# m96-chan/PyGPUkit

Measured on AMD Instinct MI355X. Metric: decode tokens/sec/GPU + prefill TFLOPS (% MFMA peak), Qwen3-0.6B bf16, higher is better.
Workload: dtype bf16

## Files before the change

pygpukit_amd/csrc/attn_core.hip.h:

```cpp
#pragma once

#include <type_traits>

#include "attn_plan.h"
#include "pgk_device.hip.h"

#ifdef PGK_PHASE_STAMPS
static __device__ unsigned long long* g_phase_tl;
#define PGK_PHASE(i)                                                                                              \
    do {                                                                                                          \
        unsigned long long* p_ = g_phase_tl;                                                                      \
        const unsigned wg_ = blockIdx.x + gridDim.x * (blockIdx.y + gridDim.y * blockIdx.z);                      \
        if (p_ && threadIdx.x == 0 && wg_ < 256u) p_[2 * (256 + 4 * wg_) + (i)] = __builtin_amdgcn_s_memrealtime(); \
    } while (0)
#else
#define PGK_PHASE(i)
#endif

namespace pgk {

template <class T> struct KVLoad;
template <> struct KVLoad<bf16> {
    __device__ static __forceinline__ void load8(const bf16* p, float (&f)[8]) {
        Vec<bf16> v; v.load(p); v.to_float(f);
// ... 186 lines not shown
        KVBatch<U> kb;
        kv_issue<D, U, NWV>(kb, kbase, vbase, p0, c1 - 1, lane);
        kv_consume<D, G, U, NWV>(kb, p0, c1, qb, lane, st);
    }
}

template <int D, int G>
__device__ __forceinline__ void decode_block_merge(const DecodeState<G>& st, float* lds, float* part,
                                                   size_t head_stride, int lane, int wid) {
    constexpr int LPR = D / 8, PPW = 64 / LPR, NS = 4 * PPW, RS = D + 2;
    const int grp = lane / LPR, sub = lane % LPR;
    const int slot = wid * PPW + grp;
#pragma unroll
    for (int g = 0; g < G; ++g) {
        float* rec = lds + ((size_t)slot * G + g) * RS;
        if (sub == 0) { rec[0] = st.m[g]; rec[1] = st.l[g]; }
#pragma unroll
        for (int j = 0; j < 8; ++j) rec[2 + sub * 8 + j] = st.o[g][j];
    }
    __syncthreads();
    for (int e = threadIdx.x; e < G * D; e += blockDim.x) {
        const int g = e / D, d = e % D;
        float mx = -INFINITY;
        for (int s = 0; s < NS; ++s) mx = fmaxf(mx, lds[((size_t)s * G + g) * RS]);
        float l = 0.f, o = 0.f;
        for (int s = 0; s < NS; ++s) {
            const float* rec = lds + ((size_t)s * G + g) * RS;
            const float w = (rec[0] == -INFINITY) ? 0.f : __expf(rec[0] - mx);
            l = fmaf(rec[1], w, l);
            o = fmaf(rec[2 + d], w, o);
        }
        float* outrec = part + (size_t)g * head_stride;
        outrec[2 + d] = o;
        if (d == 0) { outrec[0] = mx; outrec[1] = l; }
    }
}

template <int D, int G, int NWV = 4>
__device__ __forceinline__ void decode_block_merge_lds(const DecodeState<G>& st, float* lds, float* attn_out, int lane,
                                                       int wid) {
    constexpr int LPR = D / 8, PPW = 64 / LPR, NS = NWV * PPW, RS = D + 2;
    const int grp = lane / LPR, sub = lane % LPR;
    const int slot = wid * PPW + grp;
#pragma unroll
    for (int g = 0; g < G; ++g) {
        float* rec = lds + ((size_t)slot * G + g) * RS;
        if (sub == 0) { rec[0] = st.m[g]; rec[1] = st.l[g]; }
#pragma unroll
// ... 131 lines not shown
```

pygpukit_amd/csrc/engine.hip:

```cpp

#include "engine_attn.hip.h"
#include "engine_gemv.hip.h"
#include "pkgemm.hip.h"

namespace pgk {

__global__ void embed_kernel(const bf16* embed, const int32_t* tokens, float* h, int H, const int32_t* positions,
                             const float* rope_cos, const float* rope_sin, float* cur_cos, float* cur_sin, int half,
                             int max_seq) {
    const int b = blockIdx.x;
    const bf16* row = embed + (size_t)tokens[b] * H;
    for (int i = threadIdx.x; i < H; i += blockDim.x) h[(size_t)b * H + i] = to_f(row[i]);
    const int pos = min(positions[b], max_seq - 1);
    for (int i = threadIdx.x; i < half; i += blockDim.x) {
        cur_cos[(size_t)b * half + i] = rope_cos[(size_t)pos * half + i];
        cur_sin[(size_t)b * half + i] = rope_sin[(size_t)pos * half + i];
    }
}

__global__ __launch_bounds__(256) void finalize_kernel(unsigned long long* tl, const float* amax_val, const int* amax_idx, int nblk,
                                                       int32_t* tokens, int32_t* positions, int32_t* token_log,
                                                       int32_t* step_counter, int log_width, int log_cap,
                                                       const bf16* embed, float* h, int H, int bump,
                                                       unsigned long long* clk_log, const float* rope_cos,
// ... 373 lines not shown
        while (rows < rpp) rows *= 2;
        const bool tiles = rows % rpp == 0 && c.hidden_size % rows == 0 && gd / 8 <= 64;
        e->short_path = env_on("PGK_FUSED_ATTN");
        e->fused_attn = tiles && c.weight_format == 0 && (G == 1 || G == 2 || G == 4);
        e->oproj_rows = rows;
        e->attn_mfma = c.head_dim == 128 && env_on("PGK_ATTN_MFMA");
        const int nwt = c.weight_format != 0 ? 16 : 8, lpw = gd / nwt, rpp2 = lpw > 0 ? 256 / lpw : 256;
        int rows2 = c.hidden_size / 32;
        while (rows2 > 4 * rpp2 && rows2 % 2 == 0) rows2 /= 2;
        while (rows2 < rpp2) rows2 *= 2;
        e->merged_oproj = env_on("PGK_MERGED_OPROJ") && (G == 1 || G == 2 || G == 4) && lpw >= 8 && lpw <= 64 && 256 % lpw == 0 &&
                          rows2 % rpp2 == 0 && c.hidden_size % rows2 == 0 && (c.weight_format == 0 || (gd % 128 == 0 || 128 % gd == 0)) &&
                          c.weight_format != 3;
        e->moproj_rows = rows2;
    }
    const int B = c.max_batch, H = c.hidden_size, D = c.head_dim;
    pgk_status r = PGK_OK;
    auto A = [&](void** p, size_t bytes, size_t* acct) { if (r == PGK_OK) r = dev_alloc(e, p, bytes, acct); };
    const size_t kvb = (size_t)c.num_layers * e->kv_layer_elems() * sizeof(bf16);
    A((void**)&e->kcache, kvb, &e->kv_bytes);
    A((void**)&e->vcache, kvb, &e->kv_bytes);
    A((void**)&e->rope_cos, (size_t)c.max_seq_len * (D / 2) * 4, &e->ws_bytes);
    A((void**)&e->rope_sin, (size_t)c.max_seq_len * (D / 2) * 4, &e->ws_bytes);
    A((void**)&e->cur_cos, (size_t)B * (D / 2) * 4, &e->ws_bytes);
    A((void**)&e->cur_sin, (size_t)B * (D / 2) * 4, &e->ws_bytes);
    A((void**)&e->tokens, (size_t)B * 4, &e->ws_bytes);
    A((void**)&e->positions, (size_t)B * 4, &e->ws_bytes);
    A((void**)&e->token_log, (size_t)e->log_cap * B * 4, &e->ws_bytes);
    A((void**)&e->step_counter, 16, &e->ws_bytes);
    A((void**)&e->h, (size_t)B * H * 4, &e->ws_bytes);
    A((void**)&e->h2, (size_t)B * H * 4, &e->ws_bytes);
    A((void**)&e->qkv, (size_t)B * e->qkv_dim() * 4, &e->ws_bytes);
    A((void**)&e->part, (size_t)B * c.num_heads * e->nsplit * (D + 2) * 4, &e->ws_bytes);
    A((void**)&e->opart, (size_t)B * c.num_kv_heads * H * 4, &e->ws_bytes);
    A((void**)&e->act16, (size_t)B * c.intermediate_size * 2, &e->ws_bytes);
    A((void**)&e->attnv16, (size_t)B * c.num_heads * c.head_dim * 2, &e->ws_bytes);
    A((void**)&e->x16, (size_t)B * H * 2, &e->ws_bytes);
    A((void**)&e->ss_part, (size_t)64 * 1024 * 4, &e->ws_bytes);
    A((void**)&e->attnv, (size_t)B * c.num_heads * D * 4, &e->ws_bytes);
    A((void**)&e->act, (size_t)B * c.intermediate_size * 4, &e->ws_bytes);
    A((void**)&e->logits, (size_t)B * c.vocab_size * 4, &e->ws_bytes);
    e->lm_cap = e->lm_blocks > ceil_div(c.vocab_size, 16) ? e->lm_blocks : ceil_div(c.vocab_size, 16);
    {
        const char* ev = getenv("PGK_BATCHED_MFMA");
        e->batched_min = (ev && atoi(ev) == 2) ? 3 : 5;
        auto k_ok = [](int K) { return K % 128 == 0 && K <= 4096; };
        e->batched_mfma = !(ev && atoi(ev) == 0) && k_ok(c.hidden_size) && k_ok(c.intermediate_size) && k_ok(c.num_heads * c.head_dim) &&
                          c.weight_format != 3;
// ... 519 lines not shown
```

pygpukit_amd/csrc/engine_attn.hip.h:

```cpp
#pragma once

#include "attn_core.hip.h"
#include "engine_state.hip.h"

namespace pgk {

struct AttnArgs {
    const float* qkv;
    int qkv_ld;
    const bf16 *q_gamma, *k_gamma;
    float eps;
    const float *rope_cos, *rope_sin;
    bf16 *kcache, *vcache;
    const int32_t* positions;
    int hq, hkv, max_seq;
    int span;
    float scale;
    float* part;
    int nsplit;
    float* attn_direct;
    const bf16* w_o;
    const bf16* w_o_scale;
    int H, rows_per_block;
    float* opart;
    bf16* attn_direct16;
    int g_total, g_off;
};

template <int D, int G>
struct NewToken {
    float qf[G][8], kn[8], vn[8];
    uint4 qb[G], kbits, vbits;
};

template <int G>
struct NewTokenRaw {
    float4 lo[G + 2], hi[G + 2];
    uint4 gq, gk;
    float4 cs[2], sn[2];
};

template <int D, int G>
__device__ __forceinline__ void new_token_load(const AttnArgs& a, int b, int kvh, int lane, NewTokenRaw<G>& r) {
    constexpr int LPR = D / 8, HALF = D / 2;
    const int sub = lane % LPR;
    const float* row = a.qkv + (size_t)b * a.qkv_ld;
#pragma unroll
    for (int g = 0; g < G + 2; ++g) {
        const unsigned eoff = (g < G) ? (unsigned)(kvh * a.g_total + a.g_off + g) * D : (g == G ? (unsigned)(a.hq + kvh) * D : (unsigned)(a.hq + a.hkv + kvh) * D);
        r.lo[g] = *reinterpret_cast<const float4*>(row + eoff + sub * 8);
        r.hi[g] = *reinterpret_cast<const float4*>(row + eoff + sub * 8 + 4);
    }
    r.gq = r.gk = make_uint4(0, 0, 0, 0);
    if (a.q_gamma != nullptr) {
        r.gq = *reinterpret_cast<const uint4*>(a.q_gamma + sub * 8);
        r.gk = *reinterpret_cast<const uint4*>(a.k_gamma + sub * 8);
    }
    const int dd = (sub * 8) % HALF;
    const float* cs = a.rope_cos + (size_t)b * HALF + dd;
    const float* sn = a.rope_sin + (size_t)b * HALF + dd;
    r.cs[0] = *reinterpret_cast<const float4*>(cs); r.cs[1] = *reinterpret_cast<const float4*>(cs + 4);
    r.sn[0] = *reinterpret_cast<const float4*>(sn); r.sn[1] = *reinterpret_cast<const float4*>(sn + 4);
}

template <int D, int G>
__device__ __forceinline__ void new_token_finish(const AttnArgs& a, int lane, const NewTokenRaw<G>& r, NewToken<D, G>& t) {
    constexpr int LPR = D / 8;
    const int sub = lane % LPR;
    float raw[G + 2][8], gq[8], gk[8];
#pragma unroll
    for (int g = 0; g < G + 2; ++g) {
        raw[g][0] = r.lo[g].x; raw[g][1] = r.lo[g].y; raw[g][2] = r.lo[g].z; raw[g][3] = r.lo[g].w;
        raw[g][4] = r.hi[g].x; raw[g][5] = r.hi[g].y; raw[g][6] = r.hi[g].z; raw[g][7] = r.hi[g].w;
    }
    const bool has_norm = a.q_gamma != nullptr;
    if (has_norm) {
        WTraits<bf16>::decode(r.gq, gq);
        WTraits<bf16>::decode(r.gk, gk);
    } else {
#pragma unroll
        for (int j = 0; j < 8; ++j) gq[j] = gk[j] = 1.f;
    }
    const float csv[8] = {r.cs[0].x, r.cs[0].y, r.cs[0].z, r.cs[0].w, r.cs[1].x, r.cs[1].y, r.cs[1].z, r.cs[1].w};
    const float snv[8] = {r.sn[0].x, r.sn[0].y, r.sn[0].z, r.sn[0].w, r.sn[1].x, r.sn[1].y, r.sn[1].z, r.sn[1].w};
    auto norm_rope = [&](const float (&xin)[8], const float (&gamma)[8], float (&o)[8]) {
        float x[8];
#pragma unroll
        for (int j = 0; j < 8; ++j) x[j] = xin[j];
        if (has_norm) {
            float ss = 0.f;
#pragma unroll
            for (int j = 0; j < 8; ++j) ss = fmaf(x[j], x[j], ss);
            ss = group_sum<LPR>(ss);
            const float inv = 1.0f / sqrtf(ss / D + a.eps);
#pragma unroll
            for (int j = 0; j < 8; ++j) x[j] = x[j] * inv * gamma[j];
        }
        const bool lo = sub < LPR / 2;
#pragma unroll
        for (int j = 0; j < 8; ++j) {
            const float other = xor_half<LPR>(x[j]);
            o[j] = lo ? (x[j] * csv[j] - other * snv[j]) : (x[j] * csv[j] + other * snv[j]);
        }
    };
#pragma unroll
    for (int g = 0; g < G; ++g) {
        norm_rope(raw[g], gq, t.qf[g]);
#pragma unroll
        for (int j = 0; j < 8; ++j) t.qf[g][j] *= a.scale;
        Vec<bf16> qv;
        qv.from_float(t.qf[g]);
        qv.to_float(t.qf[g]);
        t.qb[g] = qv.raw;
    }
    norm_rope(raw[G], gk, t.kn);
#pragma unroll
    for (int j = 0; j < 8; ++j) t.vn[j] = raw[G + 1][j];
    Vec<bf16> kb, vb;
    kb.from_float(t.kn);
    vb.from_float(t.vn);
    kb.to_float(t.kn);
    vb.to_float(t.vn);
    t.kbits = kb.raw;
    t.vbits = vb.raw;
}

template <int D, int G>
__device__ __forceinline__ void prepare_new_token(const AttnArgs& a, int b, int kvh, int pos, int lane, NewToken<D, G>& t) {
    NewTokenRaw<G> r;
    new_token_load<D, G>(a, b, kvh, lane, r);
    new_token_finish<D, G>(a, lane, r, t);
}

template <int D, int G>
__device__ __forceinline__ void fold_new_token(const NewToken<D, G>& t, DecodeState<G>& st) {
    constexpr int LPR = D / 8;
    float s[G];
#pragma unroll
    for (int g = 0; g < G; ++g) {
        float dsum = 0.f;
#pragma unroll
        for (int j = 0; j < 8; ++j) dsum = fmaf(t.qf[g][j], t.kn[j], dsum);
        dsum = group_sum<LPR>(dsum);
        s[g] = dsum;
    }
    st.update(s, t.vn);
}

template <int D, int G, bool DIRECT>
__global__ __launch_bounds__(256) void attn_decode_kernel(unsigned long long* tl, AttnArgs a) {
    const TLStamp tls(tl);
    constexpr int LPR = D / 8, PPW = 64 / LPR, RS = D + 2;
    __shared__ __attribute__((aligned(16))) float lds[4 * PPW * G * RS];
    __shared__ float attn_out[DIRECT ? G * D : 1];
    const int lane = threadIdx.x & 63, wid = threadIdx.x >> 6, sub = lane % LPR;
    const int kvh = blockIdx.y, b = blockIdx.z;
    const size_t head_off = (((size_t)b * a.hkv + kvh) * a.max_seq) * D;
    if constexpr (DIRECT) {
        constexpr int U0 = 8, UB = 4;
        NewTokenRaw<G> raw;
        new_token_load<D, G>(a, b, kvh, lane, raw);
        __builtin_amdgcn_sched_barrier(0);
        KVBatch<U0> kb0;
        kv_issue<D, U0, 4>(kb0, a.kcache + head_off, a.vcache + head_off, wid * PPW, a.max_seq - 1, lane);
        __builtin_amdgcn_sched_barrier(0);
        const int pos = load_uniform_i32(a.positions + b);
        const int c1 = min(pos, a.max_seq);
        KVBatch<UB> kb1;
        kv_issue<D, UB, 4>(kb1, a.kcache + head_off, a.vcache + head_off, U0 * 4 * PPW + wid * PPW, max(c1 - 1, 0), lane);
        __builtin_amdgcn_sched_barrier(0);
        NewToken<D, G> t;
        new_token_finish<D, G>(a, lane, raw, t);
        if (pos < a.max_seq && wid == 0 && lane < LPR && a.g_off == 0) {
            *reinterpret_cast<uint4*>(a.kcache + head_off + (size_t)pos * D + sub * 8) = t.kbits;
            *reinterpret_cast<uint4*>(a.vcache + head_off + (size_t)pos * D + sub * 8) = t.vbits;
        }
        DecodeState<G> st;
        st.init();
        kv_consume<D, G, U0, 4>(kb0, wid * PPW, c1, t.qb, lane, st);
        kv_consume<D, G, UB, 4>(kb1, U0 * 4 * PPW + wid * PPW, c1, t.qb, lane, st);
        if (c1 > (U0 + UB) * 4 * PPW) decode_walk_trips<D, G>(a.kcache + head_off, a.vcache + head_off, (U0 + UB) * 4 * PPW, c1, t.qb, lane, wid, st);
        if (pos < a.max_seq && wid == 0 && lane < LPR) fold_new_token<D, G>(t, st);
        decode_block_merge_lds<D, G>(st, lds, attn_out, lane, wid);
        if (a.attn_direct16) {
            for (int e = threadIdx.x; e < G * D; e += 256) a.attn_direct16[((size_t)b * a.hq + (size_t)kvh * a.g_total + a.g_off) * D + e] = from_f<bf16>(attn_out[e]);
        } else {
            for (int e = threadIdx.x; e < G * D; e += 256) a.attn_direct[((size_t)b * a.hq + (size_t)kvh * a.g_total + a.g_off) * D + e] = attn_out[e];
        }
        tls.end();
        return;
    }
    constexpr int U1 = 8;
    const int chunk = decode_chunk_len(a.span, a.nsplit, 4 * PPW);
    const int c0 = (int)blockIdx.x * chunk;
    NewTokenRaw<G> raw;
    new_token_load<D, G>(a, b, kvh, lane, raw);
    __builtin_amdgcn_sched_barrier(0);
    KVBatch<U1> kb0;
    kv_issue<D, U1, 4>(kb0, a.kcache + head_off, a.vcache + head_off, c0 + wid * PPW, a.max_seq - 1, lane);
    __builtin_amdgcn_sched_barrier(0);
    const int pos = load_uniform_i32(a.positions + b);
    const int ctx = min(pos + 1, a.max_seq);
    tls.phase(0);
    NewToken<D, G> t;
    new_token_finish<D, G>(a, lane, raw, t);
    tls.phase(1);
    const bool last_slice = (int)blockIdx.x == a.nsplit - 1;
    const int c1 = last_slice ? ctx : min(c0 + chunk, ctx);
    const bool owns_new = (pos < a.max_seq) && (pos >= c0) && (last_slice || pos < c0 + chunk);
    if (owns_new && wid == 0 && lane < LPR && a.g_off == 0) {
        *reinterpret_cast<uint4*>(a.kcache + head_off + (size_t)pos * D + sub * 8) = t.kbits;
        *reinterpret_cast<uint4*>(a.vcache + head_off + (size_t)pos * D + sub * 8) = t.vbits;
    }
    DecodeState<G> st;
    st.init();
    const int cend = owns_new ? min(c1, pos) : c1;
    kv_consume<D, G, U1, 4>(kb0, c0 + wid * PPW, cend, t.qb, lane, st);
    if (cend > c0 + U1 * 4 * PPW)
        decode_walk_trips<D, G>(a.kcache + head_off, a.vcache + head_off, c0 + U1 * 4 * PPW, cend, t.qb, lane, wid, st);
    if (owns_new && wid == 0 && lane < LPR) fold_new_token<D, G>(t, st);
    tls.phase(2);
    if constexpr (DIRECT) {
        decode_block_merge_lds<D, G>(st, lds, attn_out, lane, wid);
        for (int e = threadIdx.x; e < G * D; e += 256) a.attn_direct[((size_t)b * a.hq + (size_t)kvh * a.g_total + a.g_off) * D + e] = attn_out[e];
    } else {
        decode_block_merge<D, G>(st, lds, a.part + (((size_t)b * a.hq + (size_t)kvh * a.g_total + a.g_off) * a.nsplit + blockIdx.x) * RS,
                                 (size_t)a.nsplit * RS, lane, wid);
    }
    tls.end();
}

template <int D>
__global__ void attn_merge_kernel(unsigned long long* tl, const float* part, float* attn, int hq, int nsplit) {
    const TLStamp tls(tl);
    __shared__ float w_s[64];
    __shared__ float inv_l;
    const int h = blockIdx.x, b = blockIdx.y, d = threadIdx.x;
    const float* recs = part + ((size_t)b * hq + h) * nsplit * (D + 2);
    if (threadIdx.x < 64) {
        const int s = threadIdx.x;
        const int sc = min(s, nsplit - 1);
        float m = recs[(size_t)sc * (D + 2)], l = recs[(size_t)sc * (D + 2) + 1];
        if (s >= nsplit) { m = -INFINITY; l = 0.f; }
        const float mx = wave_max(m);
        const float w = (m == -INFINITY) ? 0.f : __expf(m - mx);
        const float tot = wave_sum(w * l);
        w_s[s] = w;
        if (s == 0) inv_l = tot > 0.f ? 1.0f / tot : 0.f;
    }
    __syncthreads();
    float o = 0.f;
// ... 415 lines not shown
                uint4 w = (p < PRE) ? pre[p < PRE ? p : 0] : load_nt16(wbase + (size_t)row * ldw);
                float wf[8];
                WTraits<bf16>::decode(w, wf);
                float acc = 0.f;
#pragma unroll
                for (int j = 0; j < 8; ++j) acc = fmaf(wf[j], xf[j], acc);
                acc = group_sum<LPW>(acc);
                if (lr == 0) outp[row] = acc;
            }
        }
    } else {
        const size_t ob = ((size_t)b * a.hq + (size_t)kvh * G) * D;
        if (a.attn_direct16) {
            for (int e = threadIdx.x; e < GD; e += 256) a.attn_direct16[ob + e] = from_f<bf16>(attn[e]);
        } else {
            for (int e = threadIdx.x; e < GD; e += 256) a.attn_direct[ob + e] = attn[e];
        }
    }
    tls.phase(4);
    tls.end();
}

template <int D, int G, bool FP8>
__global__ __launch_bounds__(256) void attn_merge_oproj_kernel(unsigned long long* tl, AttnArgs a) {
    const TLStamp tls(tl);
    constexpr int RS = D + 2, GD = G * D;
    constexpr int NWT = FP8 ? 16 : 8;
    constexpr int LPW = GD / NWT;
    constexpr int RPP = 256 / LPW;
    constexpr int PRE = 4;
    static_assert(LPW <= 64 && 256 % LPW == 0, "row slice must fit a wave");
    __shared__ float w_s[G][64];
    __shared__ float inv_l[G];
    __shared__ __attribute__((aligned(16))) float attn[GD];
    const int lane = threadIdx.x & 63, wid = __builtin_amdgcn_readfirstlane(threadIdx.x >> 6);
    const int kvh = blockIdx.x % a.hkv, rb = blockIdx.x / a.hkv, b = blockIdx.z;
    const int r0 = rb * a.rows_per_block;
    const int lr = threadIdx.x % LPW, rip = threadIdx.x / LPW;
    const int npass = a.rows_per_block / RPP;
    const int ldw = a.hq * D;
    const int col0 = kvh * GD + lr * NWT;
    const char* wbase = reinterpret_cast<const char*>(a.w_o) + (size_t)col0 * (FP8 ? 1 : 2);
    const size_t row_bytes = (size_t)ldw * (FP8 ? 1 : 2);
    const float* hrecs = a.part + ((size_t)b * a.hq + (size_t)kvh * G) * a.nsplit * RS;
    float m = -INFINITY, l = 0.f;
    if (wid < G) {
        const int sc = min(lane, a.nsplit - 1);
        m = hrecs[((size_t)wid * a.nsplit + sc) * RS];
        l = hrecs[((size_t)wid * a.nsplit + sc) * RS + 1];
    }
    constexpr int EPT = (GD + 255) / 256, RPRE = 32;
    float rv[EPT][RPRE];
#pragma unroll
    for (int i = 0; i < EPT; ++i) {
        const int e = min((int)threadIdx.x + 256 * i, GD - 1), g = e / D, d = e % D;
        const float* recs = hrecs + (size_t)g * a.nsplit * RS + 2 + d;
#pragma unroll
        for (int u = 0; u < RPRE; ++u) rv[i][u] = recs[(size_t)min(u, a.nsplit - 1) * RS];
    }
    __builtin_amdgcn_sched_barrier(0);
    uint4 pre[PRE];
    float psc[PRE];
#pragma unroll
    for (int p = 0; p < PRE; ++p) {
        const int row = r0 + min(p, npass - 1) * RPP + rip;
        pre[p] = load_nt16(wbase + (size_t)row * row_bytes);
        if constexpr (FP8) psc[p] = to_f(a.w_o_scale[(size_t)(row >> 7) * (ldw >> 7) + (col0 >> 7)]);
    }
    __builtin_amdgcn_sched_barrier(0);
    tls.phase(0);
    if (wid < G) {
        if (lane >= a.nsplit) { m = -INFINITY; l = 0.f; }
        const float mx = wave_max(m);
        const float w = (m == -INFINITY) ? 0.f : __expf(m - mx);
        const float tot = wave_sum(w * l);
        w_s[wid][lane] = w;
        if (lane == 0) inv_l[wid] = tot > 0.f ? 1.0f / tot : 0.f;
    }
    __syncthreads();
    tls.phase(1);
#pragma unroll
    for (int i = 0; i < EPT; ++i) {
        const int e = (int)threadIdx.x + 256 * i;
        if (e < GD) {
            const int g = e / D, d = e % D;
            const float* recs = hrecs + (size_t)g * a.nsplit * RS;
            float o = 0.f;
#pragma unroll
            for (int u = 0; u < RPRE; ++u) o = fmaf(u < a.nsplit ? w_s[g][u] : 0.f, rv[i][u], o);
            for (int s2 = RPRE; s2 < a.nsplit; ++s2) o = fmaf(w_s[g][s2], recs[(size_t)s2 * RS + 2 + d], o);
            attn[e] = o * inv_l[g];
        }
    }
    __syncthreads();
    tls.phase(2);
    float xf[NWT];
#pragma unroll
    for (int i = 0; i < NWT / 4; ++i) {
        const float4 u = *reinterpret_cast<const float4*>(attn + lr * NWT + 4 * i);
        xf[4 * i] = u.x; xf[4 * i + 1] = u.y; xf[4 * i + 2] = u.z; xf[4 * i + 3] = u.w;
    }
    float* outp = a.opart + ((size_t)b * a.hkv + kvh) * a.H;
    for (int p = 0; p < npass; ++p) {
        const int row = r0 + p * RPP + rip;
        uint4 w;
        float sc = 1.f;
        if (p < PRE) {
            w = pre[p < PRE ? p : 0];
            if constexpr (FP8) sc = psc[p < PRE ? p : 0];
        } else {
            w = load_nt16(wbase + (size_t)row * row_bytes);
            if constexpr (FP8) sc = to_f(a.w_o_scale[(size_t)(row >> 7) * (ldw >> 7) + (col0 >> 7)]);
        }
        float wf[NWT];
        if constexpr (FP8) WTraits<fp8e4m3>::decode(w, wf);
        else WTraits<bf16>::decode(w, wf);
        float acc = 0.f;
#pragma unroll
        for (int j = 0; j < NWT; ++j) acc = fmaf(wf[j], xf[j], acc);
        acc = group_sum<LPW>(acc * sc);
        if (lr == 0) outp[row] = acc;
    }
    tls.end();
}

template <int G, bool OPROJ = true>
static hipError_t launch_attn_mfma(dim3 grid, hipStream_t st, const AttnArgs& a) {
    constexpr int lds = 2 * AM_CHUNK * 256;
    static bool attr = false;
    if (!attr) {
        const hipError_t he = hipFuncSetAttribute(reinterpret_cast<const void*>(&attn_oproj_mfma_kernel<G, OPROJ>), hipFuncAttributeMaxDynamicSharedMemorySize, lds);
        if (he != hipSuccess) return he;
        attr = true;
    }
    if (a.hq != G * a.hkv || a.g_total != G || a.g_off != 0 || a.qkv_ld != (a.hq + 2 * a.hkv) * 128) return hipErrorInvalidValue;
    return launch_k<8>(attn_oproj_mfma_kernel<G, OPROJ>, grid, dim3(256), lds, st, a.qkv, a.kcache, a.rope_cos, a.rope_sin, a.q_gamma, a.k_gamma, a.hkv, a.max_seq, a);
}

template <class F>
static hipError_t with_group(int G, F f) {
    return G == 1 ? f(std::integral_constant<int, 1>{}) : G == 2 ? f(std::integral_constant<int, 2>{}) : G == 4 ? f(std::integral_constant<int, 4>{}) : hipSuccess;
}

template <int D, int G>
static hipError_t launch_attn_decode(bool direct, dim3 grid, hipStream_t st, const AttnArgs& a) {
    return direct ? launch_k(attn_decode_kernel<D, G, true>, grid, dim3(256), 0, st, a) : launch_k(attn_decode_kernel<D, G, false>, grid, dim3(256), 0, st, a);
}

enum AttnKernel { AK_FUSED_MFMA = 0, AK_FUSED_DOT2, AK_DIRECT_MFMA, AK_DIRECT, AK_SPLIT };
enum AttnTail { AT_NONE = 0, AT_MERGE, AT_MERGE_OPROJ_BF16, AT_MERGE_OPROJ_FP8 };
struct AttnChoice { AttnKernel kernel; AttnTail tail; int nsplit, span; bool out_bf16; };
inline AttnChoice attn_choice(const Engine* e, int m, int step_span, const AttnFlags& f) {
    const auto& c = e->cfg;
    const int D = c.head_dim, G = c.num_heads / c.num_kv_heads;
    AttnChoice ch{};
    ch.span = (step_span > 0 && step_span < c.max_seq_len) ? step_span : c.max_seq_len;
    int ns = e->cu_count * (m >= 4 ? 2 : 1) / (c.num_kv_heads * m);
    const int ns_cap = ceil_div(ch.span, 64) < e->nsplit ? ceil_div(ch.span, 64) : e->nsplit;
    ns = ns < 1 ? 1 : (ns > ns_cap ? ns_cap : ns);
    ch.nsplit = f.direct ? 1 : ceil_div(ch.span, decode_chunk_len(ch.span, ns, 4 * (64 / (D / 8))));
    ch.out_bf16 = f.direct && f.direct_bf16;
    if (!group_instantiated(G)) ch.kernel = f.direct ? AK_DIRECT : AK_SPLIT;
    else if (f.fused) ch.kernel = (D == 128 && e->attn_mfma) ? AK_FUSED_MFMA : AK_FUSED_DOT2;
    else if (f.direct) ch.kernel = (D == 128 && e->attn_mfma && m * (int)c.num_kv_heads <= e->cu_count) ? AK_DIRECT_MFMA : AK_DIRECT;
    else ch.kernel = AK_SPLIT;
    const bool f8 = c.weight_format == 1 || c.weight_format == 2;
    ch.tail = f.merged ? (f8 ? AT_MERGE_OPROJ_FP8 : AT_MERGE_OPROJ_BF16) : ((!f.fused && !f.direct) ? AT_MERGE : AT_NONE);
    return ch;
}
// ... 40 lines not shown
            a.g_off = off;
            he = with_group(gc, [&](auto g) { return launch_attn_decode<D, decltype(g)::value>(direct, grid, st, a); });
            PGK_CHECK_HIP(he);
            ++*cx.launches;
            off += gc;
        }
    } else {
        he = with_group(G, [&](auto g) {
            constexpr int GG = decltype(g)::value;
            if constexpr (D == 128) {
                if (pick.kernel == AK_FUSED_MFMA) return launch_attn_mfma<GG>(dim3(c.num_kv_heads, c.hidden_size / e->oproj_rows, m), st, a);
                if (pick.kernel == AK_DIRECT_MFMA) return launch_attn_mfma<GG, false>(dim3(c.num_kv_heads, 1, m), st, a);
            }
            if (pick.kernel == AK_FUSED_DOT2) return launch_k(attn_oproj_kernel<D, GG>, grid, dim3(256), 0, st, a);
            return launch_attn_decode<D, GG>(pick.kernel == AK_DIRECT, grid, st, a);
        });
        PGK_CHECK_HIP(he);
        ++*cx.launches;
    }
    if (pick.tail == AT_MERGE_OPROJ_BF16 || pick.tail == AT_MERGE_OPROJ_FP8) {
        PGK_REQUIRE(!fused && !direct && group_instantiated(G), "engine: merged o_proj on an unsupported attention path");
        mark(KC_OPROJ);
        a.rows_per_block = e->moproj_rows;
        const dim3 g2((c.hidden_size / e->moproj_rows) * c.num_kv_heads, 1, m);
        PGK_REQUIRE(c.weight_format != 3, "engine: merged o_proj has no NVF4 form");
        const bool f8 = pick.tail == AT_MERGE_OPROJ_FP8;
        he = with_group(G, [&](auto g) {
            constexpr int GG = decltype(g)::value;
            return f8 ? launch_k(attn_merge_oproj_kernel<D, GG, true>, g2, dim3(256), 0, st, a) : launch_k(attn_merge_oproj_kernel<D, GG, false>, g2, dim3(256), 0, st, a);
        });
        PGK_CHECK_HIP(he);
        ++*cx.launches;
    } else if (pick.tail == AT_MERGE) {
        PGK_CHECK_HIP(launch_k(attn_merge_kernel<D>, dim3(c.num_heads, m), dim3(D), 0, st, (const float*)a.part,
                               e->attnv + (size_t)b0 * c.num_heads * D, (int)c.num_heads, (int)a.nsplit));
        ++*cx.launches;
    }
    return PGK_OK;
}

static pgk_status launch_attn(const StepCtx& cx, int layer, const AttnFlags& af) {
    return cx.e->cfg.head_dim == 128 ? launch_attn_d<128>(cx, layer, af) : launch_attn_d<64>(cx, layer, af);
}

}
```

Before: 1745.

## Restructure split decode attention: per-wave new-token prep via LDS, scalar kernel args

The split decode attention kernel now takes hot fields as scalar kernel arguments, with head counts packed into one int and sin as an offset from cos. It computes the new token's q/k/v norm+RoPE by spreading items across waves and sharing them through LDS. KV loads use 32-bit byte offsets with a clamped limit, and the V request is issued right after the K request. The merged o_proj kernel gets a 2D grid, 32-bit addressing and unrolled fixed pass counts. cur_cos/cur_sin are also merged into one allocation. The aim is less address arithmetic and register pressure plus more memory-level parallelism, at the cost of an extra __syncthreads and added launch-time validation.

```diff
diff --git a/pygpukit_amd/csrc/attn_core.hip.h b/pygpukit_amd/csrc/attn_core.hip.h
--- a/pygpukit_amd/csrc/attn_core.hip.h
+++ b/pygpukit_amd/csrc/attn_core.hip.h
@@ -232,8 +232,10 @@
     for (int e = threadIdx.x; e < G * D; e += blockDim.x) {
         const int g = e / D, d = e % D;
         float mx = -INFINITY;
+#pragma unroll
         for (int s = 0; s < NS; ++s) mx = fmaxf(mx, lds[((size_t)s * G + g) * RS]);
         float l = 0.f, o = 0.f;
+#pragma unroll
         for (int s = 0; s < NS; ++s) {
             const float* rec = lds + ((size_t)s * G + g) * RS;
             const float w = (rec[0] == -INFINITY) ? 0.f : __expf(rec[0] - mx);
diff --git a/pygpukit_amd/csrc/engine.hip b/pygpukit_amd/csrc/engine.hip
--- a/pygpukit_amd/csrc/engine.hip
+++ b/pygpukit_amd/csrc/engine.hip
@@ -419,8 +419,8 @@
     A((void**)&e->vcache, kvb, &e->kv_bytes);
     A((void**)&e->rope_cos, (size_t)c.max_seq_len * (D / 2) * 4, &e->ws_bytes);
     A((void**)&e->rope_sin, (size_t)c.max_seq_len * (D / 2) * 4, &e->ws_bytes);
-    A((void**)&e->cur_cos, (size_t)B * (D / 2) * 4, &e->ws_bytes);
-    A((void**)&e->cur_sin, (size_t)B * (D / 2) * 4, &e->ws_bytes);
+    A((void**)&e->cur_cos, (size_t)2 * B * (D / 2) * 4, &e->ws_bytes);
+    if (r == PGK_OK) e->cur_sin = e->cur_cos + (size_t)B * (D / 2);
     A((void**)&e->tokens, (size_t)B * 4, &e->ws_bytes);
     A((void**)&e->positions, (size_t)B * 4, &e->ws_bytes);
     A((void**)&e->token_log, (size_t)e->log_cap * B * 4, &e->ws_bytes);
diff --git a/pygpukit_amd/csrc/engine_attn.hip.h b/pygpukit_amd/csrc/engine_attn.hip.h
--- a/pygpukit_amd/csrc/engine_attn.hip.h
+++ b/pygpukit_amd/csrc/engine_attn.hip.h
@@ -40,8 +40,18 @@
     float4 cs[2], sn[2];
 };
 
-template <int D, int G>
-__device__ __forceinline__ void new_token_load(const AttnArgs& a, int b, int kvh, int lane, NewTokenRaw<G>& r) {
+struct NewTokenSrc {
+    const float* qkv;
+    int qkv_ld, hq, hkv, g_total, g_off;
+    const bf16 *q_gamma, *k_gamma;
+    const float *rope_cos, *rope_sin;
+    static __device__ __forceinline__ NewTokenSrc of(const AttnArgs& a) {
+        return NewTokenSrc{a.qkv, a.qkv_ld, a.hq, a.hkv, a.g_total, a.g_off, a.q_gamma, a.k_gamma, a.rope_cos, a.rope_sin};
+    }
+};
+
+template <int D, int G>
+__device__ __forceinline__ void new_token_load(const NewTokenSrc& a, int b, int kvh, int lane, NewTokenRaw<G>& r) {
     constexpr int LPR = D / 8, HALF = D / 2;
     const int sub = lane % LPR;
     const float* row = a.qkv + (size_t)b * a.qkv_ld;
@@ -64,7 +74,36 @@
 }
 
 template <int D, int G>
-__device__ __forceinline__ void new_token_finish(const AttnArgs& a, int lane, const NewTokenRaw<G>& r, NewToken<D, G>& t) {
+__device__ __forceinline__ void new_token_load(const AttnArgs& a, int b, int kvh, int lane, NewTokenRaw<G>& r) {
+    new_token_load<D, G>(NewTokenSrc::of(a), b, kvh, lane, r);
+}
+
+template <int D>
+__device__ __forceinline__ void norm_rope8(const float (&xin)[8], const float (&gamma)[8], bool has_norm, float eps, const float (&csv)[8],
+                                           const float (&snv)[8], int sub, float (&o)[8]) {
+    constexpr int LPR = D / 8;
+    float x[8];
+#pragma unroll
+    for (int j = 0; j < 8; ++j) x[j] = xin[j];
+    if (has_norm) {
+        float ss = 0.f;
+#pragma unroll
+        for (int j = 0; j < 8; ++j) ss = fmaf(x[j], x[j], ss);
+        ss = group_sum<LPR>(ss);
+        const float inv = 1.0f / sqrtf(ss / D + eps);
+#pragma unroll
+        for (int j = 0; j < 8; ++j) x[j] = x[j] * inv * gamma[j];
+    }
+    const bool lo = sub < LPR / 2;
+#pragma unroll
+    for (int j = 0; j < 8; ++j) {
+        const float other = xor_half<LPR>(x[j]);
+        o[j] = lo ? (x[j] * csv[j] - other * snv[j]) : (x[j] * csv[j] + other * snv[j]);
+    }
+}
+
+template <int D, int G>
+__device__ __forceinline__ void new_token_finish(bool has_norm, float eps, float scale, int lane, const NewTokenRaw<G>& r, NewToken<D, G>& t) {
     constexpr int LPR = D / 8;
     const int sub = lane % LPR;
     float raw[G + 2][8], gq[8], gk[8];
@@ -73,7 +112,6 @@
         raw[g][0] = r.lo[g].x; raw[g][1] = r.lo[g].y; raw[g][2] = r.lo[g].z; raw[g][3] = r.lo[g].w;
         raw[g][4] = r.hi[g].x; raw[g][5] = r.hi[g].y; raw[g][6] = r.hi[g].z; raw[g][7] = r.hi[g].w;
     }
-    const bool has_norm = a.q_gamma != nullptr;
     if (has_norm) {
         WTraits<bf16>::decode(r.gq, gq);
         WTraits<bf16>::decode(r.gk, gk);
@@ -83,31 +121,12 @@
     }
     const float csv[8] = {r.cs[0].x, r.cs[0].y, r.cs[0].z, r.cs[0].w, r.cs[1].x, r.cs[1].y, r.cs[1].z, r.cs[1].w};
     const float snv[8] = {r.sn[0].x, r.sn[0].y, r.sn[0].z, r.sn[0].w, r.sn[1].x, r.sn[1].y, r.sn[1].z, r.sn[1].w};
-    auto norm_rope = [&](const float (&xin)[8], const float (&gamma)[8], float (&o)[8]) {
-        float x[8];
-#pragma unroll
-        for (int j = 0; j < 8; ++j) x[j] = xin[j];
-        if (has_norm) {
-            float ss = 0.f;
-#pragma unroll
-            for (int j = 0; j < 8; ++j) ss = fmaf(x[j], x[j], ss);
-            ss = group_sum<LPR>(ss);
-            const float inv = 1.0f / sqrtf(ss / D + a.eps);
-#pragma unroll
-            for (int j = 0; j < 8; ++j) x[j] = x[j] * inv * gamma[j];
-        }
-        const bool lo = sub < LPR / 2;
-#pragma unroll
-        for (int j = 0; j < 8; ++j) {
-            const float other = xor_half<LPR>(x[j]);
-            o[j] = lo ? (x[j] * csv[j] - other * snv[j]) : (x[j] * csv[j] + other * snv[j]);
-        }
-    };
+    auto norm_rope = [&](const float (&xin)[8], const float (&gamma)[8], float (&o)[8]) { norm_rope8<D>(xin, gamma, has_norm, eps, csv, snv, sub, o); };
 #pragma unroll
     for (int g = 0; g < G; ++g) {
         norm_rope(raw[g], gq, t.qf[g]);
 #pragma unroll
-        for (int j = 0; j < 8; ++j) t.qf[g][j] *= a.scale;
+        for (int j = 0; j < 8; ++j) t.qf[g][j] *= scale;
         Vec<bf16> qv;
         qv.from_float(t.qf[g]);
         qv.to_float(t.qf[g]);
@@ -126,6 +145,96 @@
 }
 
 template <int D, int G>
+__device__ __forceinline__ void new_token_finish(const AttnArgs& a, int lane, const NewTokenRaw<G>& r, NewToken<D, G>& t) {
+    new_token_finish<D, G>(a.q_gamma != nullptr, a.eps, a.scale, lane, r, t);
+}
+
+template <int D, int G>
+struct NewTokenShared { uint4 q[G][D / 8], k[D / 8], v[D / 8]; };
+
+template <int G>
+struct NewTokenItems {
+    static constexpr int NI = (G + 2 + 3) / 4;
+    float4 lo[NI], hi[NI];
+    uint4 gm[NI];
+    float4 cs[2], sn[2];
+};
+
+template <int D, int G>
+__device__ __forceinline__ void new_token_items_load(const NewTokenSrc& a, int b, int kvh, int lane, int wid, NewTokenItems<G>& r) {
+    constexpr int LPR = D / 8, HALF = D / 2;
+    const int sub = lane % LPR;
+    const float* row = a.qkv + (size_t)b * a.qkv_ld;
+#pragma unroll
+    for (int i = 0; i < NewTokenItems<G>::NI; ++i) {
+        const int it = min(wid + 4 * i, G + 1);
+        const unsigned eoff = (it < G) ? (unsigned)(kvh * a.g_total + a.g_off + it) * D : (it == G ? (unsigned)(a.hq + kvh) * D : (unsigned)(a.hq + a.hkv + kvh) * D);
+        r.lo[i] = *reinterpret_cast<const float4*>(row + eoff + sub * 8);
+        r.hi[i] = *reinterpret_cast<const float4*>(row + eoff + sub * 8 + 4);
+        const bf16* gp = a.q_gamma != nullptr ? (it < G ? a.q_gamma : a.k_gamma) : reinterpret_cast<const bf16*>(a.rope_cos + (size_t)b * HALF);
+        r.gm[i] = *reinterpret_cast<const uint4*>(gp + sub * 8);
+    }
+    const int dd = (sub * 8) % HALF;
+    const float* cs = a.rope_cos + (size_t)b * HALF + dd;
+    const float* sn = a.rope_sin + (size_t)b * HALF + dd;
+    r.cs[0] = *reinterpret_cast<const float4*>(cs); r.cs[1] = *reinterpret_cast<const float4*>(cs + 4);
+    r.sn[0] = *reinterpret_cast<const float4*>(sn); r.sn[1] = *reinterpret_cast<const float4*>(sn + 4);
+}
+
+template <int D, int G>
+__device__ __forceinline__ void new_token_items_publish(bool has_norm, float eps, float scale, int lane, int wid, const NewTokenItems<G>& r,
+                                                        NewTokenShared<D, G>& sh) {
+    constexpr int LPR = D / 8;
+    const int sub = lane % LPR;
+    const float csv[8] = {r.cs[0].x, r.cs[0].y, r.cs[0].z, r.cs[0].w, r.cs[1].x, r.cs[1].y, r.cs[1].z, r.cs[1].w};
+    const float snv[8] = {r.sn[0].x, r.sn[0].y, r.sn[0].z, r.sn[0].w, r.sn[1].x, r.sn[1].y, r.sn[1].z, r.sn[1].w};
+#pragma unroll
+    for (int i = 0; i < NewTokenItems<G>::NI; ++i) {
+        const int it = wid + 4 * i;
+        if (it < G + 2) {
+            float x[8] = {r.lo[i].x, r.lo[i].y, r.lo[i].z, r.lo[i].w, r.hi[i].x, r.hi[i].y, r.hi[i].z, r.hi[i].w};
+            if (it <= G) {
+                float gm[8], o[8];
+                if (has_norm) {
+                    WTraits<bf16>::decode(r.gm[i], gm);
+                } else {
+#pragma unroll
+                    for (int j = 0; j < 8; ++j) gm[j] = 1.f;
+                }
+                norm_rope8<D>(x, gm, has_norm, eps, csv, snv, sub, o);
+#pragma unroll
+                for (int j = 0; j < 8; ++j) x[j] = (it < G) ? o[j] * scale : o[j];
+            }
+            Vec<bf16> xb;
+            xb.from_float(x);
+            if (lane < LPR) {
+                if (it < G) sh.q[it][lane] = xb.raw;
+                else if (it == G) sh.k[lane] = xb.raw;
+                else sh.v[lane] = xb.raw;
+            }
+        }
+    }
+}
+
+template <int D, int G>
+__device__ __forceinline__ void new_token_from_shared(const NewTokenShared<D, G>& sh, int sub, NewToken<D, G>& t) {
+#pragma unroll
+    for (int g = 0; g < G; ++g) {
+        Vec<bf16> qv;
+        qv.raw = sh.q[g][sub];
+        qv.to_float(t.qf[g]);
+        t.qb[g] = qv.raw;
+    }
+    Vec<bf16> kb, vb;
+    kb.raw = sh.k[sub];
+    vb.raw = sh.v[sub];
+    kb.to_float(t.kn);
+    vb.to_float(t.vn);
+    t.kbits = kb.raw;
+    t.vbits = vb.raw;
+}
+
+template <int D, int G>
 __device__ __forceinline__ void prepare_new_token(const AttnArgs& a, int b, int kvh, int pos, int lane, NewToken<D, G>& t) {
     NewTokenRaw<G> r;
     new_token_load<D, G>(a, b, kvh, lane, r);
@@ -147,86 +256,111 @@
     st.update(s, t.vn);
 }
 
+template <int D, int U, int NWV>
+__device__ __forceinline__ void kv_request(uint4 (&dst)[U], const bf16* base, uint32_t off0, uint32_t lim) {
+    constexpr uint32_t STEP = NWV * (64 / (D / 8)) * D * 2;
+    const char* cb = reinterpret_cast<const char*>(base);
+#pragma unroll
+    for (int u = 0; u < U; ++u) dst[u] = *reinterpret_cast<const uint4*>(cb + min(off0 + STEP * u, lim));
+}
+
 template <int D, int G, bool DIRECT>
-__global__ __launch_bounds__(256) void attn_decode_kernel(unsigned long long* tl, AttnArgs a) {
-    const TLStamp tls(tl);
+__global__ __launch_bounds__(256) void attn_decode_kernel(const float* qkv_, bf16* kcache_, const float* rope_cos_, const bf16* q_gamma_,
+                                                          const bf16* k_gamma_, int sin_off_, int heads_, int max_seq_, int chunk_,
+                                                          unsigned long long* tl, AttnArgs a) {
+    const TLStamp tls(tl, TLStamp::Deferred{});
     constexpr int LPR = D / 8, PPW = 64 / LPR, RS = D + 2;
     __shared__ __attribute__((aligned(16))) float lds[4 * PPW * G * RS];
     __shared__ float attn_out[DIRECT ? G * D : 1];
     const int lane = threadIdx.x & 63, wid = threadIdx.x >> 6, sub = lane % LPR;
     const int kvh = blockIdx.y, b = blockIdx.z;
-    const size_t head_off = (((size_t)b * a.hkv + kvh) * a.max_seq) * D;
+    const int hkv_ = heads_ & 0xFFFF, g_total_ = (heads_ >> 16) & 0xFF, g_off_ = (heads_ >> 24) & 0xFF;
+    const int hq_ = g_total_ * hkv_;
+    const NewTokenSrc src{qkv_, (hq_ + 2 * hkv_) * D, hq_, hkv_, g_total_, g_off_, q_gamma_, k_gamma_, rope_cos_,
+                          reinterpret_cast<const float*>(reinterpret_cast<const char*>(rope_cos_) + sin_off_)};
+    const bool has_norm = q_gamma_ != nullptr;
+    const size_t head_off = (((size_t)b * hkv_ + kvh) * max_seq_) * D;
     if constexpr (DIRECT) {
         constexpr int U0 = 8, UB = 4;
         NewTokenRaw<G> raw;
-        new_token_load<D, G>(a, b, kvh, lane, raw);
+        new_token_load<D, G>(src, b, kvh, lane, raw);
         __builtin_amdgcn_sched_barrier(0);
         KVBatch<U0> kb0;
-        kv_issue<D, U0, 4>(kb0, a.kcache + head_off, a.vcache + head_off, wid * PPW, a.max_seq - 1, lane);
+        kv_issue<D, U0, 4>(kb0, kcache_ + head_off, a.vcache + head_off, wid * PPW, max_seq_ - 1, lane);
         __builtin_amdgcn_sched_barrier(0);
         const int pos = load_uniform_i32(a.positions + b);
-        const int c1 = min(pos, a.max_seq);
+        const int c1 = min(pos, max_seq_);
         KVBatch<UB> kb1;
-        kv_issue<D, UB, 4>(kb1, a.kcache + head_off, a.vcache + head_off, U0 * 4 * PPW + wid * PPW, max(c1 - 1, 0), lane);
+        kv_issue<D, UB, 4>(kb1, kcache_ + head_off, a.vcache + head_off, U0 * 4 * PPW + wid * PPW, max(c1 - 1, 0), lane);
         __builtin_amdgcn_sched_barrier(0);
         NewToken<D, G> t;
-        new_token_finish<D, G>(a, lane, raw, t);
-        if (pos < a.max_seq && wid == 0 && lane < LPR && a.g_off == 0) {
-            *reinterpret_cast<uint4*>(a.kcache + head_off + (size_t)pos * D + sub * 8) = t.kbits;
+        new_token_finish<D, G>(has_norm, a.eps, a.scale, lane, raw, t);
+        if (pos < max_seq_ && wid == 0 && lane < LPR && g_off_ == 0) {
+            *reinterpret_cast<uint4*>(kcache_ + head_off + (size_t)pos * D + sub * 8) = t.kbits;
             *reinterpret_cast<uint4*>(a.vcache + head_off + (size_t)pos * D + sub * 8) = t.vbits;
         }
         DecodeState<G> st;
         st.init();
         kv_consume<D, G, U0, 4>(kb0, wid * PPW, c1, t.qb, lane, st);
         kv_consume<D, G, UB, 4>(kb1, U0 * 4 * PPW + wid * PPW, c1, t.qb, lane, st);
-        if (c1 > (U0 + UB) * 4 * PPW) decode_walk_trips<D, G>(a.kcache + head_off, a.vcache + head_off, (U0 + UB) * 4 * PPW, c1, t.qb, lane, wid, st);
-        if (pos < a.max_seq && wid == 0 && lane < LPR) fold_new_token<D, G>(t, st);
+        if (c1 > (U0 + UB) * 4 * PPW) decode_walk_trips<D, G>(kcache_ + head_off, a.vcache + head_off, (U0 + UB) * 4 * PPW, c1, t.qb, lane, wid, st);
+        if (pos < max_seq_ && wid == 0 && lane < LPR) fold_new_token<D, G>(t, st);
         decode_block_merge_lds<D, G>(st, lds, attn_out, lane, wid);
         if (a.attn_direct16) {
-            for (int e = threadIdx.x; e < G * D; e += 256) a.attn_direct16[((size_t)b * a.hq + (size_t)kvh * a.g_total + a.g_off) * D + e] = from_f<bf16>(attn_out[e]);
+            for (int e = threadIdx.x; e < G * D; e += 256) a.attn_direct16[((size_t)b * hq_ + (size_t)kvh * g_total_ + g_off_) * D + e] = from_f<bf16>(attn_out[e]);
         } else {
-            for (int e = threadIdx.x; e < G * D; e += 256) a.attn_direct[((size_t)b * a.hq + (size_t)kvh * a.g_total + a.g_off) * D + e] = attn_out[e];
+            for (int e = threadIdx.x; e < G * D; e += 256) a.attn_direct[((size_t)b * hq_ + (size_t)kvh * g_total_ + g_off_) * D + e] = attn_out[e];
         }
         tls.end();
         return;
     }
     constexpr int U1 = 8;
-    const int chunk = decode_chunk_len(a.span, a.nsplit, 4 * PPW);
+    const int wv = __builtin_amdgcn_readfirstlane(wid);
+    const int chunk = chunk_;
     const int c0 = (int)blockIdx.x * chunk;
-    NewTokenRaw<G> raw;
-    new_token_load<D, G>(a, b, kvh, lane, raw);
+    __shared__ __attribute__((aligned(16))) NewTokenShared<D, G> nt_sh;
+    NewTokenItems<G> raw;
+    new_token_items_load<D, G>(src, b, kvh, lane, wv, raw);
     __builtin_amdgcn_sched_barrier(0);
+    const uint32_t off0 = (uint32_t)(wid * PPW + lane / LPR) * (2 * D) + (uint32_t)sub * 16;
+    const uint32_t lim = c0 + U1 * 4 * PPW <= max_seq_ ? 0xFFFFFFFFu : (uint32_t)(max_seq_ - 1 - c0) * (2 * D) + (uint32_t)sub * 16;
+    const size_t slice_off = head_off + (size_t)c0 * D;
     KVBatch<U1> kb0;
-    kv_issue<D, U1, 4>(kb0, a.kcache + head_off, a.vcache + head_off, c0 + wid * PPW, a.max_seq - 1, lane);
+    kv_request<D, U1, 4>(kb0.k, kcache_ + slice_off, off0, lim);
     __builtin_amdgcn_sched_barrier(0);
-    const int pos = load_uniform_i32(a.positions + b);
-    const int ctx = min(pos + 1, a.max_seq);
+    const int pos = *(const __attribute__((address_space(4))) int32_t*)(a.positions + b);
+    kv_request<D, U1, 4>(kb0.v, a.vcache + slice_off, off0, lim);
+    __builtin_amdgcn_sched_barrier(0);
     tls.phase(0);
-    NewToken<D, G> t;
-    new_token_finish<D, G>(a, lane, raw, t);
+    new_token_items_publish<D, G>(has_norm, a.eps, a.scale, lane, wv, raw, nt_sh);
+    __syncthreads();
+    uint4 qb[G];
+#pragma unroll
+    for (int g = 0; g < G; ++g) qb[g] = nt_sh.q[g][sub];
     tls.phase(1);
+    const int ctx = min(pos + 1, max_seq_);
     const bool last_slice = (int)blockIdx.x == a.nsplit - 1;
     const int c1 = last_slice ? ctx : min(c0 + chunk, ctx);
-    const bool owns_new = (pos < a.max_seq) && (pos >= c0) && (last_slice || pos < c0 + chunk);
-    if (owns_new && wid == 0 && lane < LPR && a.g_off == 0) {
-        *reinterpret_cast<uint4*>(a.kcache + head_off + (size_t)pos * D + sub * 8) = t.kbits;
-        *reinterpret_cast<uint4*>(a.vcache + head_off + (size_t)pos * D + sub * 8) = t.vbits;
+    const bool owns_new = (pos < max_seq_) && (pos >= c0) && (last_slice || pos < c0 + chunk);
+    const bool folds = owns_new && wid == 0 && lane < LPR;
+    NewToken<D, G> t;
+    if (folds) {
+        new_token_from_shared<D, G>(nt_sh, sub, t);
+        if (g_off_ == 0) {
+            *reinterpret_cast<uint4*>(kcache_ + head_off + (size_t)pos * D + sub * 8) = t.kbits;
+            *reinterpret_cast<uint4*>(a.vcache + head_off + (size_t)pos * D + sub * 8) = t.vbits;
+        }
     }
     DecodeState<G> st;
     st.init();
     const int cend = owns_new ? min(c1, pos) : c1;
-    kv_consume<D, G, U1, 4>(kb0, c0 + wid * PPW, cend, t.qb, lane, st);
+    kv_consume<D, G, U1, 4>(kb0, c0 + wid * PPW, cend, qb, lane, st);
     if (cend > c0 + U1 * 4 * PPW)
-        decode_walk_trips<D, G>(a.kcache + head_off, a.vcache + head_off, c0 + U1 * 4 * PPW, cend, t.qb, lane, wid, st);
-    if (owns_new && wid == 0 && lane < LPR) fold_new_token<D, G>(t, st);
+        decode_walk_trips<D, G>(kcache_ + head_off, a.vcache + head_off, c0 + U1 * 4 * PPW, cend, qb, lane, wid, st);
+    if (folds) fold_new_token<D, G>(t, st);
     tls.phase(2);
-    if constexpr (DIRECT) {
-        decode_block_merge_lds<D, G>(st, lds, attn_out, lane, wid);
-        for (int e = threadIdx.x; e < G * D; e += 256) a.attn_direct[((size_t)b * a.hq + (size_t)kvh * a.g_total + a.g_off) * D + e] = attn_out[e];
-    } else {
-        decode_block_merge<D, G>(st, lds, a.part + (((size_t)b * a.hq + (size_t)kvh * a.g_total + a.g_off) * a.nsplit + blockIdx.x) * RS,
-                                 (size_t)a.nsplit * RS, lane, wid);
-    }
+    decode_block_merge<D, G>(st, lds, a.part + (((size_t)b * hq_ + (size_t)kvh * g_total_ + g_off_) * a.nsplit + blockIdx.x) * RS,
+                             (size_t)a.nsplit * RS, lane, wid);
     tls.end();
 }
 
@@ -688,8 +822,9 @@
 }
 
 template <int D, int G, bool FP8>
-__global__ __launch_bounds__(256) void attn_merge_oproj_kernel(unsigned long long* tl, AttnArgs a) {
-    const TLStamp tls(tl);
+__global__ __launch_bounds__(256) void attn_merge_oproj_kernel(const float* part_, const void* w_o_, const bf16* w_o_scale_, float* opart_,
+                                                               int nsplit_, int hkv_, int rows_, int H_, unsigned long long* tl) {
+    const TLStamp tls(tl, TLStamp::Deferred{});
     constexpr int RS = D + 2, GD = G * D;
     constexpr int NWT = FP8 ? 16 : 8;
     constexpr int LPW = GD / NWT;
@@ -700,43 +835,45 @@
     __shared__ float inv_l[G];
     __shared__ __attribute__((aligned(16))) float attn[GD];
     const int lane = threadIdx.x & 63, wid = __builtin_amdgcn_readfirstlane(threadIdx.x >> 6);
-    const int kvh = blockIdx.x % a.hkv, rb = blockIdx.x / a.hkv, b = blockIdx.z;
-    const int r0 = rb * a.rows_per_block;
+    const int kvh = blockIdx.x, rb = blockIdx.y, b = blockIdx.z;
+    const int hq = G * hkv_;
+    const int r0 = rb * rows_;
     const int lr = threadIdx.x % LPW, rip = threadIdx.x / LPW;
-    const int npass = a.rows_per_block / RPP;
-    const int ldw = a.hq * D;
+    const int npass = rows_ / RPP;
+    const int ldw = hq * D;
     const int col0 = kvh * GD + lr * NWT;
-    const char* wbase = reinterpret_cast<const char*>(a.w_o) + (size_t)col0 * (FP8 ? 1 : 2);
-    const size_t row_bytes = (size_t)ldw * (FP8 ? 1 : 2);
-    const float* hrecs = a.part + ((size_t)b * a.hq + (size_t)kvh * G) * a.nsplit * RS;
+    const uint32_t row_bytes = (uint32_t)ldw * (FP8 ? 1 : 2);
+    const char* wbase = reinterpret_cast<const char*>(w_o_) + ((size_t)r0 * ldw + (size_t)kvh * GD) * (FP8 ? 1 : 2);
+    const uint32_t woff = (uint32_t)rip * row_bytes + (uint32_t)lr * 16;
+    const char* hrecs = reinterpret_cast<const char*>(part_ + ((size_t)b * hq + (size_t)kvh * G) * nsplit_ * RS);
     float m = -INFINITY, l = 0.f;
     if (wid < G) {
-        const int sc = min(lane, a.nsplit - 1);
-        m = hrecs[((size_t)wid * a.nsplit + sc) * RS];
-        l = hrecs[((size_t)wid * a.nsplit + sc) * RS + 1];
+        const uint32_t ro = (uint32_t)(wid * nsplit_ + min(lane, nsplit_ - 1)) * (RS * 4);
+        m = *reinterpret_cast<const float*>(hrecs + ro);
+        l = *reinterpret_cast<const float*>(hrecs + ro + 4);
     }
     constexpr int EPT = (GD + 255) / 256, RPRE = 32;
     float rv[EPT][RPRE];
 #pragma unroll
     for (int i = 0; i < EPT; ++i) {
         const int e = min((int)threadIdx.x + 256 * i, GD - 1), g = e / D, d = e % D;
-        const float* recs = hrecs + (size_t)g * a.nsplit * RS + 2 + d;
-#pragma unroll
-        for (int u = 0; u < RPRE; ++u) rv[i][u] = recs[(size_t)min(u, a.nsplit - 1) * RS];
+        const uint32_t eo = (uint32_t)(g * nsplit_ * RS + 2 + d) * 4;
+#pragma unroll
+        for (int u = 0; u < RPRE; ++u) rv[i][u] = *reinterpret_cast<const float*>(hrecs + ((uint32_t)min(u, nsplit_ - 1) * (RS * 4) + eo));
     }
     __builtin_amdgcn_sched_barrier(0);
     uint4 pre[PRE];
     float psc[PRE];
 #pragma unroll
     for (int p = 0; p < PRE; ++p) {
-        const int row = r0 + min(p, npass - 1) * RPP + rip;
-        pre[p] = load_nt16(wbase + (size_t)row * row_bytes);
-        if constexpr (FP8) psc[p] = to_f(a.w_o_scale[(size_t)(row >> 7) * (ldw >> 7) + (col0 >> 7)]);
+        const int pp = min(p, npass - 1);
+        pre[p] = load_nt16(wbase + ((uint32_t)pp * RPP * row_bytes + woff));
+        if constexpr (FP8) psc[p] = to_f(w_o_scale_[(size_t)((r0 + pp * RPP + rip) >> 7) * (ldw >> 7) + (col0 >> 7)]);
     }
     __builtin_amdgcn_sched_barrier(0);
     tls.phase(0);
     if (wid < G) {
-        if (lane >= a.nsplit) { m = -INFINITY; l = 0.f; }
+        if (lane >= nsplit_) { m = -INFINITY; l = 0.f; }
         const float mx = wave_max(m);
         const float w = (m == -INFINITY) ? 0.f : __expf(m - mx);
         const float tot = wave_sum(w * l);
@@ -750,11 +887,11 @@
         const int e = (int)threadIdx.x + 256 * i;
         if (e < GD) {
             const int g = e / D, d = e % D;
-            const float* recs = hrecs + (size_t)g * a.nsplit * RS;
+            const float* recs = reinterpret_cast<const float*>(hrecs) + (size_t)g * nsplit_ * RS;
             float o = 0.f;
 #pragma unroll
-            for (int u = 0; u < RPRE; ++u) o = fmaf(u < a.nsplit ? w_s[g][u] : 0.f, rv[i][u], o);
-            for (int s2 = RPRE; s2 < a.nsplit; ++s2) o = fmaf(w_s[g][s2], recs[(size_t)s2 * RS + 2 + d], o);
+            for (int u = 0; u < RPRE; ++u) o = fmaf(u < nsplit_ ? w_s[g][u] : 0.f, rv[i][u], o);
+            for (int s2 = RPRE; s2 < nsplit_; ++s2) o = fmaf(w_s[g][s2], recs[(size_t)s2 * RS + 2 + d], o);
             attn[e] = o * inv_l[g];
         }
     }
@@ -766,26 +903,47 @@
         const float4 u = *reinterpret_cast<const float4*>(attn + lr * NWT + 4 * i);
         xf[4 * i] = u.x; xf[4 * i + 1] = u.y; xf[4 * i + 2] = u.z; xf[4 * i + 3] = u.w;
     }
-    float* outp = a.opart + ((size_t)b * a.hkv + kvh) * a.H;
-    for (int p = 0; p < npass; ++p) {
-        const int row = r0 + p * RPP + rip;
-        uint4 w;
-        float sc = 1.f;
-        if (p < PRE) {
-            w = pre[p < PRE ? p : 0];
-            if constexpr (FP8) sc = psc[p < PRE ? p : 0];
-        } else {
-            w = load_nt16(wbase + (size_t)row * row_bytes);
-            if constexpr (FP8) sc = to_f(a.w_o_scale[(size_t)(row >> 7) * (ldw >> 7) + (col0 >> 7)]);
-        }
+    float* outp = opart_ + ((size_t)b * hkv_ + kvh) * H_;
+    auto pass_dot = [&](const uint4& w, float sc) {
         float wf[NWT];
         if constexpr (FP8) WTraits<fp8e4m3>::decode(w, wf);
         else WTraits<bf16>::decode(w, wf);
         float acc = 0.f;
 #pragma unroll
         for (int j = 0; j < NWT; ++j) acc = fmaf(wf[j], xf[j], acc);
-        acc = group_sum<LPW>(acc * sc);
-        if (lr == 0) outp[row] = acc;
+        return acc * sc;
+    };
+    auto wo_fixed = [&](auto np_c) {
+        constexpr int NP = decltype(np_c)::value;
+        static_assert(NP <= PRE, "every pass of a fixed count is preloaded");
+        float acc[NP];
+#pragma unroll
+        for (int p = 0; p < NP; ++p) acc[p] = pass_dot(pre[p], FP8 ? psc[p] : 1.f);
+#pragma unroll
+        for (int p = 0; p < NP; ++p) acc[p] = group_sum<LPW>(acc[p]);
+        if (lr == 0) {
+#pragma unroll
+            for (int p = 0; p < NP; ++p) outp[r0 + p * RPP + rip] = acc[p];
+        }
+    };
+    if (npass == 4) wo_fixed(std::integral_constant<int, 4>{});
+    else if (npass == 2) wo_fixed(std::integral_constant<int, 2>{});
+    else if (npass == 1) wo_fixed(std::integral_constant<int, 1>{});
+    else {
+        for (int p = 0; p < npass; ++p) {
+            const int row = r0 + p * RPP + rip;
+            uint4 w;
+            float sc = 1.f;
+            if (p < PRE) {
+                w = pre[p < PRE ? p : 0];
+                if constexpr (FP8) sc = psc[p < PRE ? p : 0];
+            } else {
+                w = load_nt16(wbase + (size_t)p * RPP * row_bytes + woff);
+                if constexpr (FP8) sc = to_f(w_o_scale_[(size_t)(row >> 7) * (ldw >> 7) + (col0 >> 7)]);
+            }
+            const float acc = group_sum<LPW>(pass_dot(w, sc));
+            if (lr == 0) outp[row] = acc;
+        }
     }
     tls.end();
 }
@@ -810,7 +968,17 @@
 
 template <int D, int G>
 static hipError_t launch_attn_decode(bool direct, dim3 grid, hipStream_t st, const AttnArgs& a) {
-    return direct ? launch_k(attn_decode_kernel<D, G, true>, grid, dim3(256), 0, st, a) : launch_k(attn_decode_kernel<D, G, false>, grid, dim3(256), 0, st, a);
+    const ptrdiff_t sin_off = reinterpret_cast<const char*>(a.rope_sin) - reinterpret_cast<const char*>(a.rope_cos);
+    if (a.hkv < 1 || a.hkv > 0xFFFF || a.g_total < G || a.g_total > 0xFF || a.g_off < 0 || a.g_off + G > a.g_total ||
+        a.hq != a.g_total * a.hkv || a.qkv_ld != (a.hq + 2 * a.hkv) * D || sin_off != (ptrdiff_t)(int)sin_off || a.nsplit < 1)
+        return hipErrorInvalidValue;
+    const int chunk = decode_chunk_len(a.span, a.nsplit, 4 * (64 / (D / 8)));
+    if (!direct && (long long)(a.nsplit - 1) * chunk >= a.max_seq) return hipErrorInvalidValue;
+    const int heads = a.hkv | (a.g_total << 16) | (a.g_off << 24);
+    auto go = [&](auto kernel) {
+        return launch_k<9>(kernel, grid, dim3(256), 0, st, a.qkv, a.kcache, a.rope_cos, a.q_gamma, a.k_gamma, (int)sin_off, heads, a.max_seq, chunk, a);
+    };
+    return direct ? go(attn_decode_kernel<D, G, true>) : go(attn_decode_kernel<D, G, false>);
 }
 
 enum AttnKernel { AK_FUSED_MFMA = 0, AK_FUSED_DOT2, AK_DIRECT_MFMA, AK_DIRECT, AK_SPLIT };
@@ -897,12 +1065,16 @@
         PGK_REQUIRE(!fused && !direct && group_instantiated(G), "engine: merged o_proj on an unsupported attention path");
         mark(KC_OPROJ);
         a.rows_per_block = e->moproj_rows;
-        const dim3 g2((c.hidden_size / e->moproj_rows) * c.num_kv_heads, 1, m);
+        const dim3 g2(c.num_kv_heads, c.hidden_size / e->moproj_rows, m);
         PGK_REQUIRE(c.weight_format != 3, "engine: merged o_proj has no NVF4 form");
         const bool f8 = pick.tail == AT_MERGE_OPROJ_FP8;
         he = with_group(G, [&](auto g) {
             constexpr int GG = decltype(g)::value;
-            return f8 ? launch_k(attn_merge_oproj_kernel<D, GG, true>, g2, dim3(256), 0, st, a) : launch_k(attn_merge_oproj_kernel<D, GG, false>, g2, dim3(256), 0, st, a);
+            if (a.hq != GG * a.hkv) return hipErrorInvalidValue;
+            auto go = [&](auto kernel) {
+                return launch_k<8>(kernel, g2, dim3(256), 0, st, (const float*)a.part, (const void*)a.w_o, a.w_o_scale, a.opart, a.nsplit, a.hkv, a.rows_per_block, a.H);
+            };
+            return f8 ? go(attn_merge_oproj_kernel<D, GG, true>) : go(attn_merge_oproj_kernel<D, GG, false>);
         });
         PGK_CHECK_HIP(he);
         ++*cx.launches;
```

After: 1741. About the same (-0.3%).
